# viviendbk/ben-or-consensus-algorithm

Hardware: AMD Instinct MI355X
Metric: simulated node-rounds/sec at N=1024,F=341, 1–8 GPUs; % of INT/popcount roofline (higher is better)
Workload: dtype e2m1 0/1 votes -> f32 exact integer counts

## Files before the change

ben-or-consensus-algorithm_amd/benor/__init__.py:

```python
from __future__ import annotations

import ctypes
import os
import secrets
import struct
from typing import Sequence

_HERE = os.path.dirname(os.path.abspath(__file__))
LIB_PATH = os.environ.get("BENOR_LIB_PATH") or os.path.join(os.path.dirname(_HERE), "lib", "libbenor.so")

BO_OK = 0
BO_ERR_ARRAYS_DONT_MATCH = 1
BO_ERR_FAULTY_COUNT = 2
BO_ERR_INVALID_ARGUMENT = 3
BO_ERR_NO_DEVICE = 4
BO_ERR_HIP = 5
BO_ERR_OUT_OF_RANGE = 6
BO_ERR_UNSUPPORTED = 7
BO_ERR_ALREADY_STARTED = 8
BO_MODE_LOCKSTEP = 0
BO_MODE_RANDOM_DELIVERY = 1
BO_MODE_EVENT = 2
BO_MODE_RANDOM_TALLY = 3
BO_MODE_RANDOM_TALLY3 = 4
BO_MODE_CRASH_TALLY = 5
BO_MODE_CRASH_PARTIAL = 6
CRASH_TABLE_MAX_BYTES = 512 << 20
CUT_RANDOM = 0xFFFFFFFF
NEVER = 0xFFFFFFFF
BO_INIT_RANDOM = 0
BO_INIT_FIXED = 1
BO_KERNEL_NONE = -1
BO_KERNEL_BLOCKED = 0
BO_KERNEL_W = 1
BO_KERNEL_RANDOM = 2
BO_KERNEL_EVENT = 4
BO_KERNEL_LANE = 6
BO_KERNEL_MFMA = 7
BO_KERNEL_MFMA_SMALL = 8
BO_KERNEL_TALLY = 9
BO_KERNEL_TALLY3 = 10
BO_KERNEL_TALLY_CRASH = 11
BO_KERNEL_TALLY_PARTIAL = 12
KERNEL_NAMES = {BO_KERNEL_NONE: "none", BO_KERNEL_BLOCKED: "blocked popcount", BO_KERNEL_W: "W popcount",
                BO_KERNEL_RANDOM: "random delivery", BO_KERNEL_EVENT: "event level", BO_KERNEL_LANE: "lane",
                BO_KERNEL_MFMA: "matrix core (e2m1 MFMA)", BO_KERNEL_MFMA_SMALL: "packed matrix core (e2m1 MFMA, m <= 32)",
                BO_KERNEL_TALLY: "count-level random delivery (hypergeometric tallies)",
                BO_KERNEL_TALLY3: "count-level random delivery, three vote classes (hypergeometric tally + walk)",
                BO_KERNEL_TALLY_CRASH: "count-level random delivery with crashes during the run (a table per live count)",
                BO_KERNEL_TALLY_PARTIAL: "count-level random delivery with crashes cutting a broadcast short "
                                         "(a segment of receivers per cut)"}
BO_MAX_N = 4096
BO_MAX_K = 1024

KNOBS = {
    "BENOR_NO_MFMA": "validation", "BENOR_NO_MFMA_BIG": "validation", "BENOR_BIG_FORM": "validation",
    "BENOR_COOP_BW": "validation", "BENOR_SMALL_MIN_TRIALS": "validation", "BENOR_BLOCKS_PER_CU": "tuning",
    "BENOR_EVENT_LANES_PER_CU": "tuning", "BENOR_TEST_DEFER_SEG_CAP": "test", "BENOR_TIMELINE": "diagnostic",
    "BENOR_EVENT_FORM": "validation", "BENOR_LIVE_WAVES": "tuning", "BENOR_EVENT_STATS": "diagnostic",
}

BASE_NODE_PORT = 3000
DEFAULT_K_MAX = 64

EXPORTED_SYMBOLS = (
    "bo_network_create", "bo_consensus_start", "bo_consensus_stop", "bo_node_stop",
    "bo_get_state", "bo_status", "bo_network_size", "bo_network_destroy", "bo_hist_len",
    "bo_plan_create", "bo_plan_launch", "bo_plan_run", "bo_plan_popc_words_per_node_round",
    "bo_plan_live_nodes", "bo_plan_destroy", "bo_run_trials", "bo_run_trial_states",
    "bo_popc_peak", "bo_last_error", "bo_abi_version", "bo_kernel_version", "bo_plan_kernel", "bo_kernel_for",
    "bo_mfma_peak", "bo_consensus_start_sched", "bo_plan_check",
    "bo_consensus_start_live", "bo_consensus_wait", "bo_live_stop_events", "bo_get_states", "bo_consensus_poll",
    "bo_tally_cdf",
)


class Error(Exception):
    """The reference's `new Error(message)` (launchNodes.ts:11,13)."""


class AlreadyStartedError(RuntimeError):
    """libbenor error 8: a second start on one network (its inboxes persist, node.ts:29-30)."""


class NodeStateC(ctypes.Structure):
    _fields_ = [("killed", ctypes.c_int8), ("x", ctypes.c_int8), ("decided", ctypes.c_int8),
                ("pad", ctypes.c_int8), ("k", ctypes.c_int32)]


class TrialsCfgC(ctypes.Structure):
    _fields_ = [("N", ctypes.c_uint32), ("F", ctypes.c_uint32), ("k_max", ctypes.c_uint32),
                ("init_mode", ctypes.c_uint32), ("mode", ctypes.c_uint32), ("crash_cut", ctypes.c_uint32),
                ("seed", ctypes.c_uint64), ("faulty", ctypes.POINTER(ctypes.c_uint8)),
                ("init", ctypes.POINTER(ctypes.c_int8)), ("crash_at", ctypes.POINTER(ctypes.c_uint32)),
                ("crash_count", ctypes.c_uint32), ("crash_window", ctypes.c_uint32)]


def _crash_array(N, crash_at):
    if crash_at is None:
        return None
    return (ctypes.c_uint32 * max(1, N))(*[NEVER if v is None else int(v) for v in crash_at])


_lib = None


def lib() -> ctypes.CDLL:
    global _lib
    if _lib is not None:
        return _lib
    if not os.path.exists(LIB_PATH):
        raise RuntimeError(f"libbenor.so not built at {LIB_PATH}: run __graft_entry__.build()")
    L = ctypes.CDLL(LIB_PATH)
    P = ctypes.POINTER
    L.bo_network_create.argtypes = [ctypes.c_uint32, ctypes.c_uint32, ctypes.c_char_p, ctypes.c_uint32,
                                    ctypes.c_char_p, ctypes.c_uint32, P(ctypes.c_void_p)]
    L.bo_consensus_start.argtypes = [ctypes.c_void_p, ctypes.c_uint64, ctypes.c_uint32]
    L.bo_consensus_start_sched.argtypes = [ctypes.c_void_p, ctypes.c_uint64, ctypes.c_uint32, P(ctypes.c_uint32),
                                           ctypes.c_uint32]
    L.bo_consensus_start_live.argtypes = [ctypes.c_void_p, ctypes.c_uint64, ctypes.c_uint32]
    L.bo_consensus_wait.argtypes = [ctypes.c_void_p]
    L.bo_live_stop_events.argtypes = [ctypes.c_void_p, P(ctypes.c_uint32), ctypes.c_uint32]
    L.bo_consensus_stop.argtypes = [ctypes.c_void_p]
    L.bo_node_stop.argtypes = [ctypes.c_void_p, ctypes.c_uint32]
    L.bo_get_state.argtypes = [ctypes.c_void_p, ctypes.c_uint32, P(NodeStateC)]
    L.bo_get_states.argtypes = [ctypes.c_void_p, P(NodeStateC), ctypes.c_uint32, P(ctypes.c_uint64)]
    L.bo_consensus_poll.argtypes = [ctypes.c_void_p, P(ctypes.c_int)]
    L.bo_status.argtypes = [ctypes.c_void_p, ctypes.c_uint32]
    L.bo_network_size.argtypes = [ctypes.c_void_p]
    L.bo_network_size.restype = ctypes.c_uint32
    L.bo_network_destroy.argtypes = [ctypes.c_void_p]
    L.bo_network_destroy.restype = None
    L.bo_hist_len.argtypes = [ctypes.c_uint32]
    L.bo_hist_len.restype = ctypes.c_uint32
    L.bo_plan_create.argtypes = [P(TrialsCfgC), P(ctypes.c_void_p)]
    L.bo_plan_launch.argtypes = [ctypes.c_void_p, ctypes.c_uint64, ctypes.c_uint64, ctypes.c_void_p,
                                 ctypes.c_void_p]
    L.bo_plan_run.argtypes = [ctypes.c_void_p, ctypes.c_uint64, ctypes.c_uint64, P(ctypes.c_uint64)]
    L.bo_plan_check.argtypes = [ctypes.c_void_p]
    L.bo_plan_popc_words_per_node_round.argtypes = [ctypes.c_void_p]
    L.bo_plan_popc_words_per_node_round.restype = ctypes.c_uint64
    L.bo_plan_live_nodes.argtypes = [ctypes.c_void_p]
    L.bo_plan_live_nodes.restype = ctypes.c_uint32
    L.bo_plan_destroy.argtypes = [ctypes.c_void_p]
    L.bo_plan_destroy.restype = None
    L.bo_run_trials.argtypes = [P(TrialsCfgC), ctypes.c_uint64, ctypes.c_uint64, P(ctypes.c_uint64)]
    L.bo_run_trial_states.argtypes = [P(TrialsCfgC), ctypes.c_uint64, P(NodeStateC), P(ctypes.c_uint32)]
    L.bo_popc_peak.argtypes = [ctypes.c_uint32]
    L.bo_popc_peak.restype = ctypes.c_double
    L.bo_mfma_peak.argtypes = [ctypes.c_uint32]
    L.bo_mfma_peak.restype = ctypes.c_double
    L.bo_plan_kernel.argtypes = [ctypes.c_void_p]
    L.bo_plan_kernel.restype = ctypes.c_int
    L.bo_kernel_for.argtypes = [P(TrialsCfgC), P(ctypes.c_int)]
    L.bo_tally_cdf.argtypes = [ctypes.c_uint32, ctypes.c_uint32, ctypes.c_uint32, P(ctypes.c_uint32),
                               P(ctypes.c_uint64), ctypes.c_uint32, P(ctypes.c_uint32)]
    L.bo_last_error.restype = ctypes.c_char_p
    L.bo_abi_version.restype = ctypes.c_int
    L.bo_kernel_version.restype = ctypes.c_char_p
    _lib = L
    return L


def last_error() -> str:
    return lib().bo_last_error().decode()


def _check(rc: int) -> None:
    if rc != BO_OK:
        msg = last_error()
        if rc in (BO_ERR_ARRAYS_DONT_MATCH, BO_ERR_FAULTY_COUNT):
            raise Error(msg)
        if rc == BO_ERR_ALREADY_STARTED:
            raise AlreadyStartedError(f"libbenor error {rc}: {msg}")
        raise RuntimeError(f"libbenor error {rc}: {msg}")


_VAL = {0: 0, 1: 1, "?": 2}
_UNVAL = {-1: None, 0: 0, 1: 1, 2: "?"}


def _state_dict(s: NodeStateC) -> dict:
    return {"killed": bool(s.killed), "x": _UNVAL[s.x],
            "decided": None if s.decided < 0 else bool(s.decided),
            "k": None if s.k < 0 else int(s.k)}


_REC = struct.Struct("bbbbi")


def _state_dicts(arr, n: int) -> list[dict]:
    raw = memoryview(arr).cast("B").cast("Q")[:n]
    tab = {}
    for v in set(raw):
        kl, x, dec, _, k = _REC.unpack(v.to_bytes(8, "little"))
        tab[v] = {"killed": kl != 0, "x": _UNVAL[x], "decided": None if dec < 0 else dec != 0,
                  "k": None if k < 0 else k}
    return [tab[v].copy() for v in raw]


class Node:
    __slots__ = ("_net", "node_id")

    def __init__(self, net: "Network", node_id: int):
        self._net, self.node_id = net, node_id

    @property
    def port(self) -> int:
        return BASE_NODE_PORT + self.node_id

    def close(self, cb=None):
        if cb is not None:
            cb()

    def closeAllConnections(self):
        return None

    def getState(self) -> dict:
        return self._net.get_state(self.node_id)

    def status(self) -> tuple[int, str]:
        return self._net.status(self.node_id)


class Network:

    def __init__(self, N: int, F: int, initialValues: Sequence, faultyList: Sequence[bool]):
        L = lib()
        n_init, n_f = len(initialValues), len(faultyList)
        init = bytes(_VAL.get(v, -2) & 0xFF for v in initialValues) or b"\0"
        fl = bytes(v is True for v in faultyList) or b"\0"
        h = ctypes.c_void_p()
        _check(L.bo_network_create(N, F, init, n_init, fl, n_f, ctypes.byref(h)))
        self._h = h
        self.N, self.F = N, F

    def __del__(self):
        h = getattr(self, "_h", None)
        if h and _lib is not None:
            _lib.bo_network_destroy(h)
            self._h = None

    def start(self, seed: int | None = None, k_max: int = DEFAULT_K_MAX, stop_after=None) -> None:
        if seed is None:
            seed = secrets.randbits(64)
        if not stop_after:
            _check(lib().bo_consensus_start(self._h, seed, k_max))
            return
        if not isinstance(stop_after, dict) and len(stop_after) != self.N:
            raise ValueError(f"stop_after: a sequence must have N = {self.N} entries, got {len(stop_after)}")
        sched = [None] * self.N
        for i, v in (stop_after.items() if isinstance(stop_after, dict) else enumerate(stop_after)):
            if isinstance(i, bool) or not isinstance(i, int) or not 0 <= i < self.N:
                raise ValueError(f"stop_after: node {i!r} is not a node id in [0, {self.N})")
            if v is not None and (isinstance(v, bool) or not isinstance(v, int) or not 0 <= v < NEVER):
                raise ValueError(f"stop_after[{i}]: {v!r} is not a delivery count (uint32 < 2^32 - 1) or None")
            sched[i] = v
        arr = _crash_array(self.N, sched)
        _check(lib().bo_consensus_start_sched(self._h, seed, k_max, arr, self.N))

    def start_live(self, seed: int | None = None, k_max: int = DEFAULT_K_MAX) -> None:
        if seed is None:
            seed = secrets.randbits(64)
        _check(lib().bo_consensus_start_live(self._h, seed, k_max))

    def wait(self) -> None:
        _check(lib().bo_consensus_wait(self._h))

    def live_stop_events(self) -> list:
        out = (ctypes.c_uint32 * max(1, self.N))()
        _check(lib().bo_live_stop_events(self._h, out, self.N))
        return [None if v == NEVER else int(v) for v in out[:self.N]]

    def stop(self) -> None:
        _check(lib().bo_consensus_stop(self._h))

    def stop_node(self, i: int) -> None:
        _check(lib().bo_node_stop(self._h, i))

    def poll(self) -> bool:
        r = ctypes.c_int(0)
        _check(lib().bo_consensus_poll(self._h, ctypes.byref(r)))
        return bool(r.value)

    def get_state(self, i: int) -> dict:
        s = NodeStateC()
        _check(lib().bo_get_state(self._h, i, ctypes.byref(s)))
        return _state_dict(s)

    def get_states_at(self) -> tuple[list, int | None]:
        st = (NodeStateC * max(1, self.N))()
        ev = ctypes.c_uint64(0)
        _check(lib().bo_get_states(self._h, st, self.N, ctypes.byref(ev)))
        return _state_dicts(st, self.N), (None if ev.value == 2 ** 64 - 1 else int(ev.value))

    def get_states(self) -> list[dict]:
        return self.get_states_at()[0]

    def status(self, i: int) -> tuple[int, str]:
        code = lib().bo_status(self._h, i)
        if code < 0:
            _check(-code)
        return (500, "faulty") if code == 500 else (200, "live")


_current: Network | None = None


def launchNetwork(N: int, F: int, initialValues: Sequence, faultyList: Sequence[bool]) -> list[Node]:
    global _current
    net = Network(N, F, initialValues, faultyList)
    _current = net
    return [Node(net, i) for i in range(N)]


def _net(N: int) -> Network:
    if _current is None or _current.N != N:
        raise RuntimeError(f"no launched network of size {N}")
    return _current


def startConsensus(N: int, seed: int | None = None, k_max: int = DEFAULT_K_MAX, stop_after=None,
                   strict: bool = False, live: bool | None = None, sync: bool = False) -> None:
    if N == 0:
        return
    if live and stop_after:
        raise ValueError("stop_after and live are exclusive: a live run takes /stop as it comes")
    if live and sync:
        raise ValueError("live and sync are exclusive")
    if live is False:
        sync = True
    try:
        if not stop_after and not sync:
            _net(N).start_live(seed, k_max)
        else:
            _net(N).start(seed, k_max, stop_after)
    except AlreadyStartedError:
        if strict:
            raise


def stopConsensus(N: int) -> None:
    if N == 0:
        return
    _net(N).stop()


def getNodeState(nodeId: int) -> dict:
    if _current is None:
        raise RuntimeError("no launched network")
    return _current.get_state(nodeId)


def getNodesState(N: int) -> list[dict]:
    return _net(N).get_states()


def waitConsensus(N: int) -> None:
    if N == 0:
        return
    _net(N).wait()

# ... 136 lines not shown
```

ben-or-consensus-algorithm_amd/csrc/benor_mfma.h:

```cpp
#pragma once

#include "benor_device.h"

namespace benor {

typedef int mf_v4i __attribute__((ext_vector_type(4)));
typedef int mf_v8i __attribute__((ext_vector_type(8)));
typedef float mf_v16f __attribute__((ext_vector_type(16)));

template <int SA = 0>
__device__ __forceinline__ mf_v16f mfma_count(mf_v4i a, mf_v4i b, mf_v16f c) {
  const mf_v8i a8 = __builtin_shufflevector(a, a, 0, 1, 2, 3, -1, -1, -1, -1);
  const mf_v8i b8 = __builtin_shufflevector(b, b, 0, 1, 2, 3, -1, -1, -1, -1);
  return __builtin_amdgcn_mfma_scale_f32_32x32x64_f8f6f4(a8, b8, c, 4, 4, 0, 127 + SA, 0, 127);
}

__device__ __forceinline__ uint32_t sign_bytes(float e0, float e1, float e2, float e3) {
  const uint32_t lo = __builtin_amdgcn_perm(__float_as_uint(e1), __float_as_uint(e0), 0x0C0C0B09u);
  const uint32_t hi = __builtin_amdgcn_perm(__float_as_uint(e3), __float_as_uint(e2), 0x0B090C0Cu);
  return lo | hi;
}

__device__ __forceinline__ uint32_t pack_signs8(const mf_v16f &acc, int base) {
  const uint32_t s0 = sign_bytes(acc[base + 0], acc[base + 1], acc[base + 2], acc[base + 3]);
  const uint32_t s1 = sign_bytes(acc[base + 4], acc[base + 5], acc[base + 6], acc[base + 7]);
  return (s0 & 0x02020202u) | (s1 & 0x20202020u);
}

__device__ __forceinline__ uint32_t pack_fp4_8(const mf_v16f &acc, int base) {
  uint32_t r;
  asm volatile("" : "=v"(r));
  r = __builtin_amdgcn_cvt_scalef32_pk_fp4_f32(r, acc[base + 0], acc[base + 1], 1.0f, 0);
  r = __builtin_amdgcn_cvt_scalef32_pk_fp4_f32(r, acc[base + 2], acc[base + 3], 1.0f, 1);
  r = __builtin_amdgcn_cvt_scalef32_pk_fp4_f32(r, acc[base + 4], acc[base + 5], 1.0f, 2);
  r = __builtin_amdgcn_cvt_scalef32_pk_fp4_f32(r, acc[base + 6], acc[base + 7], 1.0f, 3);
  return r;
}

__device__ __forceinline__ uint32_t half_sel(uint32_t hm, uint32_t a, uint32_t b) {
  uint32_t r;
  asm("v_bfi_b32 %0, %1, %2, %3" : "=v"(r) : "v"(hm), "v"(a), "v"(b));
  return r;
}

__device__ __forceinline__ void half_trade(const uint4 &r, uint32_t h, uint32_t (&xw)[4]) {
  uint32_t hm = 0u - h;
  asm volatile("" : "+v"(hm));
  const uint32_t keep_a = half_sel(hm, r.y, r.x), keep_b = half_sel(hm, r.w, r.z);
  const uint32_t give_a = half_sel(hm, r.x, r.y), give_b = half_sel(hm, r.z, r.w);
  const int xa = (int)(((threadIdx.x & 63u) ^ 32u) << 2);
  const uint32_t recv_a = (uint32_t)__builtin_amdgcn_ds_bpermute(xa, (int)give_a);
  const uint32_t recv_b = (uint32_t)__builtin_amdgcn_ds_bpermute(xa, (int)give_b);
  xw[0] = half_sel(hm, recv_a, keep_a);
  xw[1] = half_sel(hm, recv_b, keep_b);
  xw[2] = half_sel(hm, keep_a, recv_a);
  xw[3] = half_sel(hm, keep_b, recv_b);
}

__device__ __forceinline__ mf_v4i expand_votes(uint32_t w) {
  return mf_v4i{(int)((w << 1) & 0x22222222u), (int)(w & 0x22222222u), (int)((w >> 1) & 0x22222222u),
                (int)((w >> 2) & 0x22222222u)};
}

template <int W, bool HALF, int KIND>
__global__ void __launch_bounds__(256) benor_mfma_kernel(KParams p) {
  constexpr int MT = 2 * W - (HALF ? 1 : 0);
  constexpr int KP = (MT + 1) / 2;
  constexpr int NB = (W + 1) / 2;
  constexpr int NJ = (NB + 1) / 2;
  constexpr bool SURE = KIND == 0;
  extern __shared__ __attribute__((aligned(16))) unsigned char smem[];
  const uint32_t lane = threadIdx.x & 63u, h = lane >> 5;
  const uint32_t wv = (uint32_t)__builtin_amdgcn_readfirstlane((int)(threadIdx.x >> 6));
  const uint32_t cont = SURE ? 0u : p.cont_round;
  uint32_t m = p.m, hist_len = p.hist_len;
  uint32_t trial_count = cont ? *p.trial_list_len : (uint32_t)p.trial_count;
  asm volatile("" : "+s"(m), "+s"(hist_len), "+s"(trial_count));

  uint32_t *lhist = reinterpret_cast<uint32_t *>(smem);
  uint32_t *keys = reinterpret_cast<uint32_t *>(smem + p.hist_bytes - kParamBytes);
  for (uint32_t i = threadIdx.x; i < hist_len; i += blockDim.x) lhist[i] = 0u;
  if (threadIdx.x == 0) {
    keys[0] = (uint32_t)p.seed;
    keys[1] = (uint32_t)(p.seed >> 32);
    keys[2] = (uint32_t)p.trial_begin;
    keys[3] = (uint32_t)(p.trial_begin >> 32);
  }
  __syncthreads();

  const bool random_init = p.init_mode == BO_INIT_RANDOM;
  const uint32_t M1 = cont ? m : m - p.init_q;
  const float bias_r = SURE ? -((float)(M1 >> 1) + 0.5f) : -8.0f * (float)M1;
  const float bias_p = SURE ? -((float)p.F + 0.5f) : (KIND == 2 ? 0.0f : 3.0f - 6.0f * (float)(m - 2u * p.F));
  const float dec_thr = 6.0f * (float)(2u * p.F - m) + 3.0f;
  mf_v16f cr, cp, cp_tail;
  const uint32_t mrem = m - 32u * (uint32_t)(MT - 1);
  uint32_t tail0 = 0, tail1 = 0;
#pragma unroll
  for (int j = 0; j < 16; ++j) {
    const uint32_t row = (uint32_t)((j & 3) + 8 * (j >> 2)) + 4u * h;
    const bool live = row < mrem;
    cr[j] = bias_r;
    cp[j] = bias_p;
    cp_tail[j] = live ? bias_p : __builtin_nanf("");
    const uint32_t nib = !live ? 0u : SURE ? ((j & 4) ? 0x20u : 0x02u) << (8 * (j & 3)) : 0xFu << (4 * (j & 7));
    if (j < 8) tail0 |= nib;
    else tail1 |= nib;
  }
  uint32_t fixed_w[W];
  if (!random_init) {
#pragma unroll
    for (int c = 0; c < W; ++c) {
      const uint4 q = p.init_plane[c];
      fixed_w[c] = h ? q.w : q.z;
    }
  }
  const int last_bits = (int)m - 32 * (2 * (W - 1) + (int)h);
  const uint32_t last_mask = last_bits >= 32 ? ~0u : (last_bits <= 0 ? 0u : ((1u << last_bits) - 1u));

  mf_v4i ones = {0x22222222, 0x22222222, 0x22222222, 0x22222222};
  uint32_t f_all = 0, f_1 = 0, f_2 = 0;
  const uint32_t ngroups = (trial_count + 31u) >> 5;
  const uint32_t waves_total = gridDim.x * kWavesPerBlock;
  const uint32_t wave_id = blockIdx.x * kWavesPerBlock + wv;
  uint32_t n_def = 0;
  uint32_t *seg = SURE ? nullptr : p.defer_seg + (size_t)wave_id * p.defer_seg_cap;
  for (uint32_t g = wave_id; g < ngroups; g += waves_total) {
    const uint32_t t = (g << 5) + (lane & 31u);
    const bool valid = t < trial_count;
    const uint32_t toff = cont ? (valid ? p.trial_list[t] : 0u) : t;
    uint32_t xw[W];
    if (SURE ? false : cont != 0u) {
      const uint64_t trial = lds_u64(keys + 2) + toff;
      const uint2 kk = lds_keys(keys);
#pragma unroll
      for (int c = 0; c < W; ++c) {
        const uint4 r = coin_block(kk.x, kk.y, (uint32_t)trial, (uint32_t)(trial >> 32), 32u * (2u * c + h), cont - 1u);
        xw[c] = coin_word(r, cont - 1u);
      }
    } else if (random_init) {
      const uint64_t trial = lds_u64(keys + 2) + t;
      const uint2 kk = lds_keys(keys);
#pragma unroll
      for (int j = 0; j < NJ; ++j) {
        const uint4 r = philox4x32_10(kk.x, kk.y,
                                      make_uint4((uint32_t)trial, (uint32_t)(trial >> 32), 2u * j + h, kStreamInit << 24));
        uint32_t q4[4];
        half_trade(r, h, q4);
#pragma unroll
        for (int q = 0; q < 4; ++q)
          if (4 * j + q < W) xw[4 * j + q] = q4[q];
      }
    } else {
#pragma unroll
      for (int c = 0; c < W; ++c) xw[c] = fixed_w[c];
    }
    xw[W - 1] &= last_mask;
    mf_v4i bx[W];
#pragma unroll
    for (int c = 0; c < W; ++c) bx[c] = expand_votes(xw[c]);

    uint32_t bp[MT][2];
    uint32_t qz = 0u;
    if constexpr (SURE && W <= 4) {
      __builtin_amdgcn_s_setprio(1);
      mf_v16f racc[2];
#pragma unroll
      for (int i = 0; i <= MT; ++i) {
        if (i < MT) {
          asm volatile("" : "+v"(ones));
          mf_v16f acc = mfma_count(ones, bx[0], cr);
#pragma unroll
          for (int c = 1; c < W; ++c) acc = mfma_count(ones, bx[c], acc);
          racc[i & 1] = acc;
        }
        if (i > 0) {
          bp[i - 1][0] = pack_signs8(racc[(i - 1) & 1], 0);
          bp[i - 1][1] = pack_signs8(racc[(i - 1) & 1], 8);
        }
        if (i < MT && i > 0) {
#pragma unroll
          for (int c = 0; c < W; ++c) {
            __builtin_amdgcn_sched_group_barrier(0x008, 1, 0);
            __builtin_amdgcn_sched_group_barrier(0x002, (16 + W - 1) / W, 0);
          }
        }
        __builtin_amdgcn_sched_barrier(0);
      }
    } else
#pragma unroll
    for (int i = 0; i < MT; ++i) {
      asm volatile("" : "+v"(ones));
      if constexpr (SURE) {
        mf_v16f acc = mfma_count(ones, bx[0], cr);
#pragma unroll
        for (int c = 1; c < W; ++c) acc = mfma_count(ones, bx[c], acc);
        bp[i][0] = pack_signs8(acc, 0);
        bp[i][1] = pack_signs8(acc, 8);
      } else {
        mf_v16f acc = mfma_count<4>(ones, bx[0], cr);
#pragma unroll
        for (int c = 1; c < W; ++c) acc = mfma_count<4>(ones, bx[c], acc);
        bp[i][0] = pack_fp4_8(acc, 0);
        bp[i][1] = pack_fp4_8(acc, 8);
        const uint32_t l0 = i == MT - 1 ? (tail0 & 0x22222222u) : 0x22222222u;
        const uint32_t l1 = i == MT - 1 ? (tail1 & 0x22222222u) : 0x22222222u;
        qz |= (~bp[i][0] & l0) | (~bp[i][1] & l1);
      }
      __builtin_amdgcn_sched_barrier(0);
    }
    bp[MT - 1][0] &= tail0;
    bp[MT - 1][1] &= tail1;
    mf_v4i pb[KP];
#pragma unroll
    for (int c = 0; c < KP; ++c)
      pb[c] = mf_v4i{(int)bp[2 * c][0], (int)bp[2 * c][1], 2 * c + 1 < MT ? (int)bp[2 * c + 1][0] : 0,
                     2 * c + 1 < MT ? (int)bp[2 * c + 1][1] : 0};

    uint32_t any1, any0, halt = (uint32_t)ballot(valid);
    if constexpr (SURE) {
      uint32_t s_or = 0u, s_and = ~0u;
      if constexpr (W <= 4) {
        mf_v16f pacc[2];
#pragma unroll
        for (int i = 0; i <= MT; ++i) {
          if (i < MT) {
            asm volatile("" : "+v"(ones));
            mf_v16f acc = mfma_count(ones, pb[0], cp);
#pragma unroll
            for (int c = 1; c < KP; ++c) acc = mfma_count(ones, pb[c], acc);
            pacc[i & 1] = acc;
          }
          if (i > 0) {
#pragma unroll
            for (int j = 0; j < 16; ++j) {
              const uint32_t u = __float_as_uint(pacc[(i - 1) & 1][j]);
              s_or |= u;
              s_and &= u;
            }
          }
          if (i < MT && i > 0) {
#pragma unroll
            for (int c = 0; c < KP; ++c) {
              __builtin_amdgcn_sched_group_barrier(0x008, 1, 0);
              __builtin_amdgcn_sched_group_barrier(0x002, (16 + KP - 1) / KP, 0);
            }
          }
          __builtin_amdgcn_sched_barrier(0);
        }
        __builtin_amdgcn_s_setprio(0);
      } else
#pragma unroll
      for (int i = 0; i < MT; ++i) {
        asm volatile("" : "+v"(ones));
        mf_v16f acc = mfma_count(ones, pb[0], cp);
#pragma unroll
        for (int c = 1; c < KP; ++c) acc = mfma_count(ones, pb[c], acc);
#pragma unroll
        for (int j = 0; j < 16; ++j) {
          const uint32_t u = __float_as_uint(acc[j]);
          s_or |= u;
          s_and &= u;
        }
        asm volatile("" : "+v"(s_or), "+v"(s_and));
        __builtin_amdgcn_sched_barrier(0);
      }
      const uint64_t b1 = ballot(s_or >> 31);
      const uint64_t b0 = ballot(!(s_and >> 31));
      any1 = (uint32_t)b1 | (uint32_t)(b1 >> 32);
      any0 = (uint32_t)b0 | (uint32_t)(b0 >> 32);
    } else {
      float mn = __builtin_inff(), mx = -__builtin_inff(), ma = __builtin_inff();
#pragma unroll
      for (int i = 0; i < MT; ++i) {
        asm volatile("" : "+v"(ones));
        mf_v16f acc = mfma_count(ones, pb[0], i < MT - 1 ? cp : cp_tail);
#pragma unroll
        for (int c = 1; c < KP; ++c) acc = mfma_count(ones, pb[c], acc);
#pragma unroll
        for (int j = 0; j < 16; j += 2) {
          mn = fminf(fminf(mn, acc[j]), acc[j + 1]);
          mx = fmaxf(fmaxf(mx, acc[j]), acc[j + 1]);
          if constexpr (KIND == 2) ma = fminf(fminf(ma, __builtin_fabsf(acc[j])), __builtin_fabsf(acc[j + 1]));
        }
        asm volatile("" : "+v"(mn), "+v"(mx), "+v"(ma));
        __builtin_amdgcn_sched_barrier(0);
      }
      const bool defer = qz != 0u || (KIND == 2 && !(ma > dec_thr));
      const uint64_t bd = ballot(valid && defer);
      const uint32_t dcols = (uint32_t)bd | (uint32_t)(bd >> 32);
      halt &= ~dcols;
      if (dcols) {
        if (lane < 32u && ((dcols >> lane) & 1u)) {
          const uint32_t idx = n_def + (uint32_t)__builtin_popcount(dcols & ((1u << lane) - 1u));
          if (idx < p.defer_seg_cap) seg[idx] = toff;
        }
        n_def += (uint32_t)__builtin_popcount(dcols);
      }
      const uint64_t b1 = ballot(mx > 0.0f);
      const uint64_t b0 = ballot(mn < 0.0f);
      any1 = (uint32_t)b1 | (uint32_t)(b1 >> 32);
      any0 = (uint32_t)b0 | (uint32_t)(b0 >> 32);
    }
    any1 &= halt;
    any0 &= halt;
    f_all += (uint32_t)__builtin_popcount(halt);
    f_1 += (uint32_t)__builtin_popcount(any1);
    f_2 += (uint32_t)__builtin_popcount(any1 & any0);
  }
  if constexpr (!SURE) {
    if (n_def > p.defer_seg_cap) {
      if (lane == 0) atomicOr(p.overflow, 1u);
      n_def = p.defer_seg_cap;
    }
    uint32_t *wdef = keys + 4;
    if (lane == 0) wdef[wv] = n_def;
    __syncthreads();
    uint32_t before = 0u, total = 0u;
#pragma unroll
    for (uint32_t w = 0; w < (uint32_t)kWavesPerBlock; ++w) {
      const uint32_t c = wdef[w];
      total += c;
      before += w < wv ? c : 0u;
    }
    __syncthreads();
    if (threadIdx.x == 0 && total) wdef[0] = atomicAdd(p.defer_len, total);
    __syncthreads();
    if (n_def) {
      const uint32_t base = wdef[0] + before;
      for (uint32_t i = lane; i < n_def; i += 64u) p.defer_list[base + i] = seg[i];
    }
  }

  const uint32_t rb = 3u * (cont ? cont : 1u);
  const uint32_t hc = lane == rb ? f_all - f_1 : (lane == rb + 1u ? f_1 - f_2 : (lane == rb + 2u ? f_2 : 0u));
  if (hc) atomicAdd(&lhist[lane], hc);
  if (lane == 0 && f_2) atomicAdd(&lhist[hist_len - 1u], f_2);
  __syncthreads();
  flush_hist(lhist, p);
}

template <int W, int KIND>
static inline void launch_mfma_kind(const KParams &p, int grid, hipStream_t s) {
  if (p.m <= 64u * (uint32_t)(W - 1) + 32u)
    hipLaunchKernelGGL((benor_mfma_kernel<W, true, KIND>), dim3(grid), dim3(64 * kWavesPerBlock), p.hist_bytes, s, p);
  else
    hipLaunchKernelGGL((benor_mfma_kernel<W, false, KIND>), dim3(grid), dim3(64 * kWavesPerBlock), p.hist_bytes, s, p);
}

template <int W>
hipError_t launch_mfma(const KParams &p, int grid, hipStream_t s) {
  if (p.G == 0u) launch_mfma_kind<W, 0>(p, grid, s);
  else if (p.G == 1u) launch_mfma_kind<W, 1>(p, grid, s);
  else launch_mfma_kind<W, 2>(p, grid, s);
  return hipGetLastError();
}

}
```

ben-or-consensus-algorithm_amd/csrc/benor_runtime.cpp:

```cpp
#include <hip/hip_runtime.h>

#include <cstdio>
#include <cstring>
#include <string>
#include <algorithm>
#include <utility>
#include <cstdlib>
#include <memory>
#include <mutex>
#include <thread>
#include <chrono>
#include <cmath>
#include <vector>

#include "benor.h"
#include "benor_internal.h"

namespace {

thread_local std::string g_err;

int fail(int code, const std::string &msg) {
  g_err = msg;
  return code;
}

int hip_fail(hipError_t e, const char *what) {
  g_err = std::string(what) + ": " + hipGetErrorString(e);
  return BO_ERR_HIP;
}

#define HIP_TRY(expr)                                  \
  do {                                                 \
    hipError_t e_ = (expr);                            \
    if (e_ != hipSuccess) return hip_fail(e_, #expr);  \
  } while (0)

int check_device(int *dev_out) {
  int n = 0;
  if (hipGetDeviceCount(&n) != hipSuccess || n <= 0)
    return fail(BO_ERR_NO_DEVICE, "no HIP device visible (libbenor has no CPU fallback)");
  int dev = 0;
  HIP_TRY(hipGetDevice(&dev));
  hipDeviceProp_t prop;
  HIP_TRY(hipGetDeviceProperties(&prop, dev));
  if (std::strncmp(prop.gcnArchName, "gfx950", 6) != 0)
    return fail(BO_ERR_NO_DEVICE, std::string("device is ") + prop.gcnArchName + ", libbenor targets gfx950");
  if (dev_out) *dev_out = dev;
  return BO_OK;
}

__global__ void add_bin_kernel(unsigned long long *hist, uint32_t bin, unsigned long long n) {
  if (threadIdx.x == 0 && blockIdx.x == 0) hist[bin] += n;
}

}

namespace benor {
struct KnobSpec {
  const char *name, *kind;
};
constexpr KnobSpec kKnobs[] = {
    {"BENOR_NO_MFMA", "validation"},
    {"BENOR_NO_MFMA_BIG", "validation"},
    {"BENOR_BIG_FORM", "validation"},
    {"BENOR_COOP_BW", "validation"},
    {"BENOR_SMALL_MIN_TRIALS", "validation"},
    {"BENOR_BLOCKS_PER_CU", "tuning"},
    {"BENOR_EVENT_LANES_PER_CU", "tuning"},
    {"BENOR_EVENT_FORM", "validation"},
    {"BENOR_LIVE_WAVES", "tuning"},
    {"BENOR_EVENT_STATS", "diagnostic"},
    {"BENOR_TEST_DEFER_SEG_CAP", "test"},
    {"BENOR_TIMELINE", "diagnostic"},
};

const char *knob(const char *name) {
  for (const KnobSpec &k : kKnobs)
    if (std::strcmp(k.name, name) == 0) return std::getenv(name);
  std::fprintf(stderr, "libbenor: knob %s is not registered in kKnobs\n", name);
  std::abort();
}

uint32_t knob_u32(const char *name, uint32_t dflt) {
  const char *v = knob(name);
  return v && *v ? (uint32_t)std::strtoul(v, nullptr, 10) : dflt;
}

bool knob_is(const char *name, const char *value) {
  const char *v = knob(name);
  return v && std::strcmp(v, value) == 0;
}
}

struct bo_live;
struct bo_network {
  uint32_t N = 0, F = 0;
  std::vector<bo_node_state> st;
  std::vector<uint8_t> faulty;
  bool started = false;
  bool in_flight = false;
  std::shared_ptr<bo_live> live;
  int live_rc = 0;
  std::vector<uint32_t> stop_events;
  mutable std::mutex mu;
  std::mutex wait_mu;
  std::mutex snap_mu;
};

struct bo_plan {
  benor::KParams kp{};
  bo_trials_cfg cfg{};
  std::vector<uint32_t> live_ids;
  uint32_t *d_live = nullptr;
  uint4 *d_init = nullptr;
  int8_t *d_init_x = nullptr;
  uint32_t *d_crash = nullptr;
  uint32_t *d_scratch = nullptr;
  uint32_t *d_defer = nullptr;
  uint64_t defer_words = 0;
  uint32_t *d_flag = nullptr;
  uint64_t *d_stops = nullptr;
  unsigned char *d_tally = nullptr;
  int device = 0;
};

namespace {
struct LiveSlot {
  int device = -1;
  hipStream_t s = nullptr;
  uint32_t *box = nullptr;
  uint32_t *dbox = nullptr;
  unsigned char *d = nullptr;
  size_t bytes = 0;
  unsigned char *hp = nullptr;
  size_t hp_bytes = 0;
};
constexpr size_t kSlotKeepBytes = 64u << 20;
std::mutex g_slots_mu;
std::vector<LiveSlot *> g_free_slots;

struct WgRun {
  size_t o_st = 0, o_r = 0;
  size_t o_stats = 0;
  uint32_t N = 0, F = 0;
};
}

struct bo_live {
  LiveSlot *slot = nullptr;
  WgRun run;
  std::vector<uint32_t> active;
  bool failed = false;
  std::vector<uint32_t> snap_words;
  uint64_t snap_e = 0;
  std::chrono::steady_clock::time_point snap_t{};
  bool snap_ok = false;
  ~bo_live();
};

namespace {
void live_post(bo_live *lr, const uint32_t *ids, uint32_t n) {
  uint32_t *box = lr->slot->box;
  uint32_t words[BO_MAX_N / 32] = {};
  for (uint32_t j = 0; j < n; ++j) words[ids[j] >> 5] |= 1u << (ids[j] & 31u);
  for (uint32_t w = 0; w < BO_MAX_N / 32; ++w)
    if (words[w]) __atomic_fetch_or(&box[benor::kLiveReq + w], words[w], __ATOMIC_RELAXED);
  __atomic_fetch_add(&box[0], 1u, __ATOMIC_RELEASE);
}
}

extern "C" {

const char *bo_last_error(void) { return g_err.c_str(); }
int bo_abi_version(void) { return BENOR_ABI_VERSION; }
#ifndef BENOR_KERNEL_SHA
#define BENOR_KERNEL_SHA "unknown"
#endif
const char *bo_kernel_version(void) { return BENOR_KERNEL_SHA; }
uint32_t bo_hist_len(uint32_t k_max) { return (k_max + 1u) * 3u + 1u; }

int bo_network_create(uint32_t N, uint32_t F, const int8_t *init, uint32_t n_init,
                      const uint8_t *faulty, uint32_t n_faulty, bo_network **out) {
  if (!out) return fail(BO_ERR_INVALID_ARGUMENT, "out is NULL");
  *out = nullptr;
  if (n_init != n_faulty || N != n_init) return fail(BO_ERR_ARRAYS_DONT_MATCH, "Arrays don't match");
  if (N > 0 && (!init || !faulty)) return fail(BO_ERR_INVALID_ARGUMENT, "initial_values / faulty_list is NULL");
  uint32_t cnt = 0;
  for (uint32_t i = 0; i < n_faulty; ++i) cnt += faulty[i] ? 1u : 0u;
  if (cnt != F) return fail(BO_ERR_FAULTY_COUNT, "faultyList doesnt have F faulties");
  if (N > BO_MAX_N) return fail(BO_ERR_UNSUPPORTED, "N exceeds BO_MAX_N");
  for (uint32_t i = 0; i < N; ++i)
    if (init[i] < 0 || init[i] > 2) return fail(BO_ERR_INVALID_ARGUMENT, "initial value must be 0, 1 or '?'(2)");
  auto *net = new bo_network();
  net->N = N;
  net->F = F;
  net->st.resize(N);
  net->faulty.assign(faulty, faulty + N);
  for (uint32_t i = 0; i < N; ++i) {
    const bool f = faulty[i] != 0;
    net->st[i].killed = f ? 1 : 0;
    net->st[i].x = f ? -1 : init[i];
    net->st[i].decided = f ? -1 : 0;
    net->st[i].pad = 0;
    net->st[i].k = f ? -1 : 0;
  }
  *out = net;
  return BO_OK;
}

uint32_t bo_network_size(const bo_network *net) { return net ? net->N : 0u; }

void bo_network_destroy(bo_network *net) {
  if (!net) return;
  (void)bo_consensus_wait(net);
  delete net;
}

int bo_status(const bo_network *net, uint32_t i) {
  if (!net) return -fail(BO_ERR_INVALID_ARGUMENT, "net is NULL");
  if (i >= net->N) return -fail(BO_ERR_OUT_OF_RANGE, "node index out of range");
  std::lock_guard<std::mutex> g(net->mu);
  return net->st[i].killed ? 500 : 200;
}

namespace {
int get_states_impl(bo_network *net, bo_node_state *out, uint64_t *events_out);
}

int bo_get_state(const bo_network *net, uint32_t i, bo_node_state *out) {
  if (!net || !out) return fail(BO_ERR_INVALID_ARGUMENT, "NULL argument");
  if (i >= net->N) return fail(BO_ERR_OUT_OF_RANGE, "node index out of range");
  {
    std::lock_guard<std::mutex> g(net->mu);
    if (!net->live) {
      *out = net->st[i];
      return net->live_rc;
    }
  }
  std::vector<bo_node_state> all(net->N);
  const int rc = get_states_impl(const_cast<bo_network *>(net), all.data(), nullptr);
  *out = all[i];
  return rc;
}

int bo_node_stop(bo_network *net, uint32_t i) {
  if (!net) return fail(BO_ERR_INVALID_ARGUMENT, "net is NULL");
  if (i >= net->N) return fail(BO_ERR_OUT_OF_RANGE, "node index out of range");
  std::lock_guard<std::mutex> g(net->mu);
  net->st[i].killed = 1;
  if (net->live) live_post(net->live.get(), &i, 1u);
  return BO_OK;
}

int bo_consensus_stop(bo_network *net) {
  if (!net) return fail(BO_ERR_INVALID_ARGUMENT, "net is NULL");
  std::lock_guard<std::mutex> g(net->mu);
  for (auto &s : net->st) s.killed = 1;
  if (net->live) {
    std::vector<uint32_t> all(net->N);
    for (uint32_t i = 0; i < net->N; ++i) all[i] = i;
    live_post(net->live.get(), all.data(), net->N);
  }
  return BO_OK;
}

int bo_consensus_start(bo_network *net, uint64_t seed, uint32_t k_max) {
  return bo_consensus_start_sched(net, seed, k_max, nullptr, 0u);
}

namespace {
struct StartPlan {
  std::vector<uint8_t> crashed;
  std::vector<int8_t> x;
  std::vector<uint32_t> active, sched;
  bool scheduled = false;
  bool launch = false;
};

int start_prologue(bo_network *net, uint32_t k_max, const uint32_t *stop_after, uint32_t n_stop_after,
                   StartPlan &sp) {
  if (!net) return fail(BO_ERR_INVALID_ARGUMENT, "net is NULL");
  if (k_max < 1 || k_max > BO_MAX_K) return fail(BO_ERR_INVALID_ARGUMENT, "k_max out of range");
  const uint32_t N = net->N;
  if (stop_after && n_stop_after != N) return fail(BO_ERR_INVALID_ARGUMENT, "stop schedule must have N entries");
  sp.crashed.assign(N, 0);
  sp.x.assign(N, 0);
  sp.sched.assign(N, 0xFFFFFFFFu);
  std::lock_guard<std::mutex> g(net->mu);
  if (net->started)
    return fail(BO_ERR_ALREADY_STARTED, net->in_flight
                ? "consensus is already running on this network"
                : "consensus already started on this network: node inboxes persist across /start "
                  "(node.ts:29-30), launch a new network to run again");
  for (uint32_t i = 0; i < N; ++i) {
    sp.crashed[i] = net->st[i].killed ? 1 : 0;
    sp.x[i] = net->st[i].killed ? 0 : net->st[i].x;
    if (!net->st[i].killed) {
      sp.active.push_back(i);
      if (stop_after) sp.sched[i] = stop_after[i];
    }
  }
  for (uint32_t i : sp.active) sp.scheduled = sp.scheduled || sp.sched[i] != 0xFFFFFFFFu;
  if (sp.active.empty()) { net->started = true; return BO_OK; }
  const int64_t quorum = (int64_t)N - (int64_t)net->F;
  if ((int64_t)sp.active.size() < quorum) {
    for (uint32_t i : sp.active) net->st[i].k = 1;
    net->started = true;
    return BO_OK;
  }
  int dev = 0;
  const int rc = check_device(&dev);
  if (rc) return rc;
  net->started = true;
  net->in_flight = true;
  sp.launch = true;
  return BO_OK;
}

bo_trials_cfg start_cfg(const bo_network *net, uint64_t seed, uint32_t k_max, StartPlan &sp, int mode) {
  bo_trials_cfg cfg{};
  cfg.N = net->N;
  cfg.F = net->F;
  cfg.k_max = k_max;
  cfg.init_mode = BO_INIT_FIXED;
  cfg.mode = mode;
  cfg.seed = seed;
  cfg.faulty = sp.crashed.data();
  cfg.init = sp.x.data();
  cfg.crash_at = sp.scheduled ? sp.sched.data() : nullptr;
  return cfg;
}

void merge_states(bo_network *net, const std::vector<uint32_t> &active, const std::vector<bo_node_state> &states) {
  const uint32_t N = net->N;
  for (uint32_t i : active) {
    const int8_t killed = net->st[i].killed;
    net->st[i] = states[i];
    net->st[i].killed = (int8_t)(killed | states[i].killed);
  }
  bool all_decided = true;
  for (uint32_t i = 0; i < N; ++i) all_decided = all_decided && net->st[i].decided == 1;
  if (all_decided)
    for (uint32_t i = 0; i < N; ++i) net->st[i].killed = 1;
}
}

namespace {
int run_sched_wg(const bo_trials_cfg *cfg, std::vector<bo_node_state> &states);
}

int bo_consensus_start_sched(bo_network *net, uint64_t seed, uint32_t k_max, const uint32_t *stop_after,
                             uint32_t n_stop_after) {
  StartPlan sp;
  int rc = start_prologue(net, k_max, stop_after, n_stop_after, sp);
  if (rc || !sp.launch) return rc;
  const bo_trials_cfg cfg = start_cfg(net, seed, k_max, sp, sp.scheduled ? BO_MODE_EVENT : BO_MODE_LOCKSTEP);
  std::vector<bo_node_state> states(net->N);
  uint32_t rounds = 0;
  rc = sp.scheduled ? run_sched_wg(&cfg, states) : bo_run_trial_states(&cfg, 0, states.data(), &rounds);
  std::lock_guard<std::mutex> g(net->mu);
  net->in_flight = false;
  if (rc) {
    net->started = false;
    return rc;
  }
  merge_states(net, sp.active, states);
// ... 1074 lines not shown
```

Before: 3072 billion.

## Pack two row-tile counts into one f32 MFMA accumulator via scaled exponent

Adds a paired form of the KIND-0 matrix-core kernel. The second row tile's count is accumulated into the same f32 accumulator at a shifted bit position using the MFMA scale exponent, with integer biases chosen so threshold indicator bits land at fixed positions. This halves the number of accumulators to pack and fold, and turns the byte-sign extraction into masked permutes. It keeps the same number of MFMA issues but doubles the MFMAs per accumulator chain, so it relies on exact f32 integer range and adds a chain-latency risk. It is on by default, and BENOR_MFMA_PAIR=0 falls back to the old path.

```diff
diff --git a/ben-or-consensus-algorithm_amd/benor/__init__.py b/ben-or-consensus-algorithm_amd/benor/__init__.py
--- a/ben-or-consensus-algorithm_amd/benor/__init__.py
+++ b/ben-or-consensus-algorithm_amd/benor/__init__.py
@@ -58,6 +58,7 @@
     "BENOR_COOP_BW": "validation", "BENOR_SMALL_MIN_TRIALS": "validation", "BENOR_BLOCKS_PER_CU": "tuning",
     "BENOR_EVENT_LANES_PER_CU": "tuning", "BENOR_TEST_DEFER_SEG_CAP": "test", "BENOR_TIMELINE": "diagnostic",
     "BENOR_EVENT_FORM": "validation", "BENOR_LIVE_WAVES": "tuning", "BENOR_EVENT_STATS": "diagnostic",
+    "BENOR_MFMA_PAIR": "validation",
 }
 
 BASE_NODE_PORT = 3000
diff --git a/ben-or-consensus-algorithm_amd/csrc/benor_mfma.h b/ben-or-consensus-algorithm_amd/csrc/benor_mfma.h
--- a/ben-or-consensus-algorithm_amd/csrc/benor_mfma.h
+++ b/ben-or-consensus-algorithm_amd/csrc/benor_mfma.h
@@ -1,6 +1,7 @@
 #pragma once
 
 #include "benor_device.h"
+#include "benor_mfma_pair.h"
 
 namespace benor {
 
@@ -62,13 +63,21 @@
                 (int)((w >> 2) & 0x22222222u)};
 }
 
-template <int W, bool HALF, int KIND>
+__device__ __forceinline__ uint32_t pack_pair4(const mf_v16f &acc, int base) {
+  const uint32_t x = __builtin_amdgcn_perm(__float_as_uint(acc[base + 1]), __float_as_uint(acc[base + 0]), pairf::kSelX);
+  const uint32_t y = __builtin_amdgcn_perm(__float_as_uint(acc[base + 3]), __float_as_uint(acc[base + 2]), pairf::kSelY);
+  return (x & pairf::kMaskX) | (y & pairf::kMaskY);
+}
+
+template <int W, bool HALF, int KIND, bool PAIR = false>
 __global__ void __launch_bounds__(256) benor_mfma_kernel(KParams p) {
+  static_assert(!PAIR || KIND == 0, "the paired form is KIND 0's");
   constexpr int MT = 2 * W - (HALF ? 1 : 0);
   constexpr int KP = (MT + 1) / 2;
   constexpr int NB = (W + 1) / 2;
   constexpr int NJ = (NB + 1) / 2;
   constexpr bool SURE = KIND == 0;
+  constexpr bool PAIRED = PAIR;
   extern __shared__ __attribute__((aligned(16))) unsigned char smem[];
   const uint32_t lane = threadIdx.x & 63u, h = lane >> 5;
   const uint32_t wv = (uint32_t)__builtin_amdgcn_readfirstlane((int)(threadIdx.x >> 6));
@@ -90,8 +99,9 @@
 
   const bool random_init = p.init_mode == BO_INIT_RANDOM;
   const uint32_t M1 = cont ? m : m - p.init_q;
-  const float bias_r = SURE ? -((float)(M1 >> 1) + 0.5f) : -8.0f * (float)M1;
-  const float bias_p = SURE ? -((float)p.F + 0.5f) : (KIND == 2 ? 0.0f : 3.0f - 6.0f * (float)(m - 2u * p.F));
+  const float bias_r = PAIRED ? pairf::bias_r2(M1) : SURE ? -((float)(M1 >> 1) + 0.5f) : -8.0f * (float)M1;
+  const float bias_p = PAIRED ? pairf::bias_p2(m, p.F)
+                       : SURE ? -((float)p.F + 0.5f) : (KIND == 2 ? 0.0f : 3.0f - 6.0f * (float)(m - 2u * p.F));
   const float dec_thr = 6.0f * (float)(2u * p.F - m) + 3.0f;
   mf_v16f cr, cp, cp_tail;
   const uint32_t mrem = m - 32u * (uint32_t)(MT - 1);
@@ -106,6 +116,16 @@
     const uint32_t nib = !live ? 0u : SURE ? ((j & 4) ? 0x20u : 0x02u) << (8 * (j & 3)) : 0xFu << (4 * (j & 7));
     if (j < 8) tail0 |= nib;
     else tail1 |= nib;
+  }
+  uint32_t tailq[4] = {0u, 0u, 0u, 0u};
+  if constexpr (PAIRED) {
+#pragma unroll
+    for (int j = 0; j < 16; ++j) {
+      const uint32_t row = (uint32_t)((j & 3) + 8 * (j >> 2)) + 4u * h;
+      const bool live = row < mrem;
+      const bool live_lo = (MT & 1) ? live : true, live_hi = (MT & 1) ? false : live;
+      tailq[j >> 2] |= (live_lo ? pairf::nib_lo(j & 3) : 0u) | (live_hi ? pairf::nib_hi(j & 3) : 0u);
+    }
   }
   uint32_t fixed_w[W];
   if (!random_init) {
@@ -161,8 +181,56 @@
     for (int c = 0; c < W; ++c) bx[c] = expand_votes(xw[c]);
 
     uint32_t bp[MT][2];
+    mf_v4i pb[KP];
     uint32_t qz = 0u;
-    if constexpr (SURE && W <= 4) {
+    if constexpr (PAIRED && W <= 4) {
+      __builtin_amdgcn_s_setprio(1);
+      mf_v16f racc[2];
+#pragma unroll
+      for (int a = 0; a <= KP; ++a) {
+        constexpr int VPM = (16 + 2 * W - 1) / (2 * W);
+        if (a < KP) {
+          asm volatile("" : "+v"(ones));
+          mf_v16f acc = mfma_count(ones, bx[0], cr);
+#pragma unroll
+          for (int c = 1; c < W; ++c) acc = mfma_count(ones, bx[c], acc);
+          if (2 * a + 1 < MT) {
+            asm volatile("" : "+v"(ones));
+#pragma unroll
+            for (int c = 0; c < W; ++c) acc = mfma_count<pairf::kShiftR>(ones, bx[c], acc);
+          }
+          racc[a & 1] = acc;
+        }
+        if (a > 0) {
+#pragma unroll
+          for (int k = 0; k < 4; ++k) pb[a - 1][k] = (int)pack_pair4(racc[(a - 1) & 1], 4 * k);
+        }
+        if (a < KP && a > 0) {
+#pragma unroll
+          for (int c = 0; c < (2 * a + 1 < MT ? 2 * W : W); ++c) {
+            __builtin_amdgcn_sched_group_barrier(0x008, 1, 0);
+            __builtin_amdgcn_sched_group_barrier(0x002, VPM, 0);
+          }
+        }
+        __builtin_amdgcn_sched_barrier(0);
+      }
+    } else if constexpr (PAIRED) {
+#pragma unroll
+      for (int a = 0; a < KP; ++a) {
+        asm volatile("" : "+v"(ones));
+        mf_v16f acc = mfma_count(ones, bx[0], cr);
+#pragma unroll
+        for (int c = 1; c < W; ++c) acc = mfma_count(ones, bx[c], acc);
+        if (2 * a + 1 < MT) {
+          asm volatile("" : "+v"(ones));
+#pragma unroll
+          for (int c = 0; c < W; ++c) acc = mfma_count<pairf::kShiftR>(ones, bx[c], acc);
+        }
+#pragma unroll
+        for (int k = 0; k < 4; ++k) pb[a][k] = (int)pack_pair4(acc, 4 * k);
+        __builtin_amdgcn_sched_barrier(0);
+      }
+    } else if constexpr (SURE && W <= 4) {
       __builtin_amdgcn_s_setprio(1);
       mf_v16f racc[2];
 #pragma unroll
@@ -209,18 +277,77 @@
       }
       __builtin_amdgcn_sched_barrier(0);
     }
-    bp[MT - 1][0] &= tail0;
-    bp[MT - 1][1] &= tail1;
-    mf_v4i pb[KP];
-#pragma unroll
-    for (int c = 0; c < KP; ++c)
-      pb[c] = mf_v4i{(int)bp[2 * c][0], (int)bp[2 * c][1], 2 * c + 1 < MT ? (int)bp[2 * c + 1][0] : 0,
-                     2 * c + 1 < MT ? (int)bp[2 * c + 1][1] : 0};
+    if constexpr (PAIRED) {
+#pragma unroll
+      for (int k = 0; k < 4; ++k) pb[KP - 1][k] &= (int)tailq[k];
+    } else {
+      bp[MT - 1][0] &= tail0;
+      bp[MT - 1][1] &= tail1;
+#pragma unroll
+      for (int c = 0; c < KP; ++c)
+        pb[c] = mf_v4i{(int)bp[2 * c][0], (int)bp[2 * c][1], 2 * c + 1 < MT ? (int)bp[2 * c + 1][0] : 0,
+                       2 * c + 1 < MT ? (int)bp[2 * c + 1][1] : 0};
+    }
 
     uint32_t any1, any0, halt = (uint32_t)ballot(valid);
     if constexpr (SURE) {
       uint32_t s_or = 0u, s_and = ~0u;
-      if constexpr (W <= 4) {
+      [[maybe_unused]] auto fold_pair = [&](const mf_v16f &acc, bool lone) {
+        uint32_t a_and = ~0u;
+#pragma unroll
+        for (int j = 0; j < 16; ++j) {
+          const uint32_t u = __float_as_uint(acc[j]);
+          s_or |= u;
+          if (lone) a_and &= u;
+          else s_and &= u;
+        }
+        if (lone) s_and &= a_and | pairf::kIndPHigh;
+      };
+      if constexpr (PAIRED && W <= 4) {
+        mf_v16f pacc[2];
+#pragma unroll
+        for (int a = 0; a <= KP; ++a) {
+          constexpr int VPM = (32 + 2 * KP - 1) / (2 * KP);
+          if (a < KP) {
+            asm volatile("" : "+v"(ones));
+            mf_v16f acc = mfma_count(ones, pb[0], cp);
+#pragma unroll
+            for (int c = 1; c < KP; ++c) acc = mfma_count(ones, pb[c], acc);
+            if (2 * a + 1 < MT) {
+              asm volatile("" : "+v"(ones));
+#pragma unroll
+              for (int c = 0; c < KP; ++c) acc = mfma_count<pairf::kShiftP>(ones, pb[c], acc);
+            }
+            pacc[a & 1] = acc;
+          }
+          if (a > 0) fold_pair(pacc[(a - 1) & 1], 2 * (a - 1) + 1 >= MT);
+          if (a < KP && a > 0) {
+#pragma unroll
+            for (int c = 0; c < (2 * a + 1 < MT ? 2 * KP : KP); ++c) {
+              __builtin_amdgcn_sched_group_barrier(0x008, 1, 0);
+              __builtin_amdgcn_sched_group_barrier(0x002, VPM, 0);
+            }
+          }
+          __builtin_amdgcn_sched_barrier(0);
+        }
+        __builtin_amdgcn_s_setprio(0);
+      } else if constexpr (PAIRED) {
+#pragma unroll
+        for (int a = 0; a < KP; ++a) {
+          asm volatile("" : "+v"(ones));
+          mf_v16f acc = mfma_count(ones, pb[0], cp);
+#pragma unroll
+          for (int c = 1; c < KP; ++c) acc = mfma_count(ones, pb[c], acc);
+          if (2 * a + 1 < MT) {
+            asm volatile("" : "+v"(ones));
+#pragma unroll
+            for (int c = 0; c < KP; ++c) acc = mfma_count<pairf::kShiftP>(ones, pb[c], acc);
+          }
+          fold_pair(acc, 2 * a + 1 >= MT);
+          asm volatile("" : "+v"(s_or), "+v"(s_and));
+          __builtin_amdgcn_sched_barrier(0);
+        }
+      } else if constexpr (W <= 4) {
         mf_v16f pacc[2];
 #pragma unroll
         for (int i = 0; i <= MT; ++i) {
@@ -265,8 +392,8 @@
         asm volatile("" : "+v"(s_or), "+v"(s_and));
         __builtin_amdgcn_sched_barrier(0);
       }
-      const uint64_t b1 = ballot(s_or >> 31);
-      const uint64_t b0 = ballot(!(s_and >> 31));
+      const uint64_t b1 = ballot(PAIRED ? (s_or & pairf::kIndP) != 0u : (s_or >> 31) != 0u);
+      const uint64_t b0 = ballot(PAIRED ? (~s_and & pairf::kIndP) != 0u : !(s_and >> 31));
       any1 = (uint32_t)b1 | (uint32_t)(b1 >> 32);
       any0 = (uint32_t)b0 | (uint32_t)(b0 >> 32);
     } else {
@@ -340,17 +467,23 @@
   flush_hist(lhist, p);
 }
 
-template <int W, int KIND>
+template <int W, int KIND, bool PAIR = false>
 static inline void launch_mfma_kind(const KParams &p, int grid, hipStream_t s) {
   if (p.m <= 64u * (uint32_t)(W - 1) + 32u)
-    hipLaunchKernelGGL((benor_mfma_kernel<W, true, KIND>), dim3(grid), dim3(64 * kWavesPerBlock), p.hist_bytes, s, p);
+    hipLaunchKernelGGL((benor_mfma_kernel<W, true, KIND, PAIR>), dim3(grid), dim3(64 * kWavesPerBlock), p.hist_bytes, s, p);
   else
-    hipLaunchKernelGGL((benor_mfma_kernel<W, false, KIND>), dim3(grid), dim3(64 * kWavesPerBlock), p.hist_bytes, s, p);
+    hipLaunchKernelGGL((benor_mfma_kernel<W, false, KIND, PAIR>), dim3(grid), dim3(64 * kWavesPerBlock), p.hist_bytes, s, p);
+}
+
+template <int W>
+static inline void launch_mfma_sure(const KParams &p, int grid, hipStream_t s) {
+  if (knob_is("BENOR_MFMA_PAIR", "0")) launch_mfma_kind<W, 0, false>(p, grid, s);
+  else launch_mfma_kind<W, 0, true>(p, grid, s);
 }
 
 template <int W>
 hipError_t launch_mfma(const KParams &p, int grid, hipStream_t s) {
-  if (p.G == 0u) launch_mfma_kind<W, 0>(p, grid, s);
+  if (p.G == 0u) launch_mfma_sure<W>(p, grid, s);
   else if (p.G == 1u) launch_mfma_kind<W, 1>(p, grid, s);
   else launch_mfma_kind<W, 2>(p, grid, s);
   return hipGetLastError();
diff --git a/ben-or-consensus-algorithm_amd/csrc/benor_mfma_pair.h b/ben-or-consensus-algorithm_amd/csrc/benor_mfma_pair.h
--- /dev/null
+++ b/ben-or-consensus-algorithm_amd/csrc/benor_mfma_pair.h
@@ -0,0 +1,50 @@
+#pragma once
+
+#include <stdint.h>
+
+#if defined(__HIPCC__) || defined(__CUDACC__)
+#define BENOR_PAIR_HD __host__ __device__
+#else
+#define BENOR_PAIR_HD
+#endif
+
+namespace benor {
+namespace pairf {
+
+constexpr int kShiftR = 12;
+constexpr int kShiftP = 11;
+constexpr uint32_t kBase = 1u << 23;
+constexpr uint32_t kIndR = (1u << 9) | (1u << 21);
+constexpr uint32_t kIndP = 0x00200400u;
+constexpr uint32_t kIndPHigh = 0x00200000u;
+constexpr uint32_t kSelX = 0x06020501u, kSelY = 0x05010602u;
+constexpr uint32_t kMaskX = 0x20200202u, kMaskY = 0x02022020u;
+
+BENOR_PAIR_HD constexpr uint32_t thr_r(uint32_t M1) { return (M1 >> 1) + 1u; }
+BENOR_PAIR_HD constexpr uint32_t thr_p(uint32_t m, uint32_t F) { return m - F; }
+
+BENOR_PAIR_HD constexpr uint32_t bias_r2_int(uint32_t M1) { return kBase + ((1u << 9) - thr_r(M1)) * (1u + (1u << kShiftR)); }
+BENOR_PAIR_HD constexpr uint32_t bias_p2_int(uint32_t m, uint32_t F) {
+  return kBase + ((1u << 10) - thr_p(m, F)) * (1u + (1u << kShiftP));
+}
+BENOR_PAIR_HD constexpr float bias_r2(uint32_t M1) { return (float)bias_r2_int(M1); }
+BENOR_PAIR_HD constexpr float bias_p2(uint32_t m, uint32_t F) { return (float)bias_p2_int(m, F); }
+
+BENOR_PAIR_HD constexpr uint32_t perm_bytes(uint32_t hi, uint32_t lo, uint32_t sel) {
+  uint32_t r = 0;
+  for (int i = 0; i < 4; ++i) {
+    const uint32_t s = (sel >> (8 * i)) & 7u;
+    r |= (((s < 4u ? lo : hi) >> (8u * (s & 3u))) & 0xFFu) << (8 * i);
+  }
+  return r;
+}
+
+BENOR_PAIR_HD constexpr uint32_t pack4_model(uint32_t u0, uint32_t u1, uint32_t u2, uint32_t u3) {
+  return (perm_bytes(u1, u0, kSelX) & kMaskX) | (perm_bytes(u3, u2, kSelY) & kMaskY);
+}
+
+BENOR_PAIR_HD constexpr uint32_t nib_lo(int i) { return 0x02u << (8 * i); }
+BENOR_PAIR_HD constexpr uint32_t nib_hi(int i) { return 0x20u << (8 * ((i + 2) & 3)); }
+
+}
+}
diff --git a/ben-or-consensus-algorithm_amd/csrc/benor_runtime.cpp b/ben-or-consensus-algorithm_amd/csrc/benor_runtime.cpp
--- a/ben-or-consensus-algorithm_amd/csrc/benor_runtime.cpp
+++ b/ben-or-consensus-algorithm_amd/csrc/benor_runtime.cpp
@@ -63,6 +63,7 @@
 constexpr KnobSpec kKnobs[] = {
     {"BENOR_NO_MFMA", "validation"},
     {"BENOR_NO_MFMA_BIG", "validation"},
+    {"BENOR_MFMA_PAIR", "validation"},
     {"BENOR_BIG_FORM", "validation"},
     {"BENOR_COOP_BW", "validation"},
     {"BENOR_SMALL_MIN_TRIALS", "validation"},
```

After: 3125 billion, median of 6. +1.7%, better.
